# markkurossi/mpc

Measured on AMD Instinct MI355X. Metric: AND-gates/sec (garble+eval), AES-128 circuit batch, higher is better.
Workload: dtype u32 (AES T-table / 128-bit label XOR, integer); 1 GPU; aes_128.circ 36663 gates / 6400 AND, batch=1024 instances per GPU, 32-byte garbling key; instances_per_gpu=1024, levels=308, launches_per_garble=1, schedule=fused-flat, hash_phases=89, lds_live_labels=1053, graph=True, outputs_ok=True, device_memory=gc_dev_alloc / gc_dev_upload (C ABI); no torch in the process, gathers=0

## Files before the change

mpc_amd/csrc/plan.cpp:

```cpp
#include "plan.h"

#include <algorithm>
#include <chrono>
#include <cstdio>
#include <cstdlib>
#include <map>
#include <numeric>

namespace gc {

namespace {
struct PlanLaps {
    bool on = std::getenv("GC_TRACE") != nullptr;
    std::chrono::steady_clock::time_point t = std::chrono::steady_clock::now();
    void lap(const char *what) {
        if (!on) return;
        const auto n = std::chrono::steady_clock::now();
        std::fprintf(stderr, "[gc trace] plan: %-28s %8.3f ms\n", what, std::chrono::duration<double, std::milli>(n - t).count());
        t = n;
    }
};
}

static inline int op_class(uint8_t op) {
    switch (op) {
    case GC_AND: return 0;
    case GC_OR: return 1;
    case GC_INV: return 2;
    default: return 3;
    }
}


static void symdiff(const std::vector<uint32_t> &a, const std::vector<uint32_t> &b, std::vector<uint32_t> *o) {
    o->clear();
    size_t i = 0, j = 0;
    while (i < a.size() || j < b.size()) {
        if (j == b.size() || (i < a.size() && a[i] < b[j])) o->push_back(a[i++]);
        else if (i == a.size() || b[j] < a[i]) o->push_back(b[j++]);
        else i++, j++;
    }
}

namespace {
struct OpView {
    const uint8_t *ops;
    struct G {
        uint8_t op;
    };
    G operator[](uint32_t g) const { return G{ops[g]}; }
};
}

static void build_flat(const OpView gates, uint32_t ngates, uint32_t nwires, uint32_t ninputs, uint32_t noutputs,
                       const std::vector<uint32_t> &src0, const std::vector<uint32_t> &src1,
                       const std::vector<uint32_t> &cur, Plan *out, bool late = false) {
    Plan &p = *out;
    PlanLaps laps;
    const uint32_t NONE = 0xffffffffu;
    const uint32_t nprod = ninputs + ngates;
    std::vector<uint32_t> phase_of;
    if (late) {
        std::vector<uint32_t> early(nprod, 0);
        uint32_t last = 0;
        for (uint32_t g = 0; g < ngates; g++) {
            const uint32_t a = std::max(early[src0[g]], early[src1[g]]);
            early[ninputs + g] = op_class(gates[g].op) != 3 ? a + 1 : a;
            last = std::max(last, early[ninputs + g]);
        }
        std::vector<uint32_t> need_by(nprod, last);
        phase_of.assign(ngates, 0);
        for (uint32_t g = ngates; g-- > 0;) {
            const uint32_t pid = ninputs + g;
            uint32_t by = need_by[pid];
            if (op_class(gates[g].op) != 3) {
                phase_of[g] = std::max(by, early[pid]);
                by = phase_of[g] - 1;
            }
            need_by[src0[g]] = std::min(need_by[src0[g]], by);
            need_by[src1[g]] = std::min(need_by[src1[g]], by);
        }
    }
    std::vector<uint32_t> A(nprod, 0), Rr(nprod, 0);
    std::vector<uint8_t> is_free(nprod, 0), rpar(ngates, 0);
    std::vector<std::vector<uint32_t>> ex(ngates);
    std::map<std::vector<uint32_t>, uint32_t> sums;
    const bool two_level = std::getenv("GC_PLAN_NO_TWO_LEVEL") == nullptr;
    std::vector<uint32_t> t0, t1, tmp;
    std::vector<std::vector<uint32_t>> fx(ngates);
    std::vector<uint8_t> fdone(ngates, 0), fp(ngates, 0);
    std::vector<uint32_t> fstack, facc, fnxt, fsingles;
    auto full_of = [&](uint32_t top) {
        const uint32_t nreal = ninputs + ngates;
        fstack.assign(1, top);
        while (!fstack.empty()) {
            const uint32_t cur = fstack.back(), cg = cur - ninputs, ca = A[cur];
            if (fdone[cg]) {
                fstack.pop_back();
                continue;
            }
            auto own_c = [&](uint32_t t) { return t < nreal && is_free[t] && A[t] == ca; };
            bool ready = true;
            for (uint32_t t : ex[cg])
                if (own_c(t) && !fdone[t - ninputs]) fstack.push_back(t), ready = false;
            if (!ready) continue;
            fsingles.clear();
            for (uint32_t t : ex[cg])
                if (!own_c(t)) fsingles.push_back(t);
            facc.swap(fsingles);
            uint8_t par = rpar[cg];
            for (uint32_t t : ex[cg])
                if (own_c(t)) {
                    symdiff(facc, fx[t - ninputs], &fnxt);
                    facc.swap(fnxt);
                    par ^= fp[t - ninputs];
                }
            fx[cg] = facc;
            fp[cg] = par;
            fdone[cg] = 1;
            fstack.pop_back();
        }
    };
    for (uint32_t g = 0; g < ngates; g++) {
        const uint32_t pid = ninputs + g, s0 = src0[g], s1 = src1[g];
        const uint32_t a = std::max(A[s0], A[s1]);
        if (op_class(gates[g].op) != 3) {
            A[pid] = late ? phase_of[g] : a + 1;
            continue;
        }
        is_free[pid] = 1;
        A[pid] = a;
        auto rnd = [&](uint32_t s) { return (is_free[s] && A[s] == a) ? Rr[s] : 0u; };
        uint32_t r = std::max(std::max(rnd(s0), rnd(s1)), 1u);
        uint8_t par = gates[g].op == GC_XNOR;
        auto terms_of = [&](uint32_t s, std::vector<uint32_t> *t) {
            if (is_free[s] && A[s] == a && Rr[s] == r) {
                *t = ex[s - ninputs];
                par ^= rpar[s - ninputs];
            } else {
                t->assign(1, s);
            }
        };
        terms_of(s0, &t0);
        terms_of(s1, &t1);
        symdiff(t0, t1, &tmp);
        if (tmp.size() > kFlatMaxTerms && two_level) {
            const uint32_t nreal = ninputs + ngates;
            auto own = [&](uint32_t t) { return t < nreal && is_free[t] && A[t] == a; };
            std::vector<uint32_t> full, nxt;
            uint8_t fpar = par;
            for (uint32_t t : tmp)
                if (!own(t)) full.push_back(t);
            for (uint32_t t : tmp)
                if (own(t)) {
                    full_of(t);
                    symdiff(full, fx[t - ninputs], &nxt);
                    full.swap(nxt);
                    fpar ^= fp[t - ninputs];
                }
            std::vector<uint32_t> raw, rest;
            for (uint32_t t : full) ((t >= nreal && A[t] == a) ? rest : raw).push_back(t);
            const size_t nblocks = (raw.size() + kFlatMaxTerms - 1) / kFlatMaxTerms;
            if (rest.size() + nblocks <= kFlatMaxTerms) {
                for (size_t b0 = 0; b0 < raw.size(); b0 += kFlatMaxTerms) {
                    std::vector<uint32_t> blk(raw.begin() + (long)b0, raw.begin() + (long)std::min(raw.size(), b0 + kFlatMaxTerms));
                    if (blk.size() == 1) {
                        rest.push_back(blk[0]);
                        continue;
                    }
                    auto it = sums.find(blk);
                    if (it == sums.end() || A[it->second] > a) {
                        const uint32_t sp = (uint32_t)A.size();
                        A.push_back(a);
                        Rr.push_back(1);
                        is_free.push_back(1);
                        ex.push_back(blk);
                        rpar.push_back(0);
                        sums[blk] = sp;
                        it = sums.find(blk);
                    }
                    rest.push_back(it->second);
                }
                std::sort(rest.begin(), rest.end());
                size_t keep = 0;
                for (size_t i = 0; i < rest.size(); i++) {
                    if (i + 1 < rest.size() && rest[i] == rest[i + 1]) i++;
                    else rest[keep++] = rest[i];
                }
                rest.resize(keep);
                tmp.swap(rest);
                par = fpar;
                r = 2;
            }
        }
        if (tmp.size() > kFlatMaxTerms) {
            r += 1;
            par = gates[g].op == GC_XNOR;
            t0.assign(1, s0);
            t1.assign(1, s1);
            symdiff(t0, t1, &tmp);
        }
        Rr[pid] = r;
        rpar[g] = par;
        ex[g] = tmp;
    }
    laps.lap("flat: term lists");
    const uint32_t nprod2 = (uint32_t)A.size(), ngates2 = (uint32_t)ex.size();
    std::vector<uint8_t> need(nprod2, 0), is_output(nprod2, 0);
    std::vector<uint32_t> stack;
    for (uint32_t j = 0; j < noutputs; j++) {
        const uint32_t w = nwires - noutputs + j;
        if (cur[w] != NONE) {
            is_output[cur[w]] = 1;
            stack.push_back(cur[w]);
        }
    }
    for (uint32_t g = 0; g < ngates; g++)
        if (!is_free[ninputs + g]) {
            need[ninputs + g] = 1;
            stack.push_back(src0[g]);
            stack.push_back(src1[g]);
        }
    while (!stack.empty()) {
        const uint32_t s = stack.back();
        stack.pop_back();
        if (need[s] && (s < ninputs || !is_free[s])) continue;
        if (need[s]) continue;
        need[s] = 1;
        if (s >= ninputs && is_free[s])
            for (uint32_t t : ex[s - ninputs]) stack.push_back(t);
    }
    std::vector<uint32_t> gl;
    for (uint32_t g = 0; g < ngates2; g++)
        if (need[ninputs + g]) gl.push_back(g);
    auto key_of = [&](uint32_t g) { return ((uint64_t)A[ninputs + g] << 32) | ((uint64_t)Rr[ninputs + g] << 8); };
    auto sub_of = [&](uint32_t g) -> uint64_t {
        if (!is_free[ninputs + g]) return (uint64_t)op_class(gates[g].op);
        return 0xffu - std::min<uint64_t>(0xfeu, ex[g].size());
    };
    {
        std::vector<std::pair<uint64_t, uint32_t>> keyed(gl.size());
        for (size_t k = 0; k < gl.size(); k++) keyed[k] = {key_of(gl[k]) | sub_of(gl[k]), gl[k]};
        std::sort(keyed.begin(), keyed.end());
        for (size_t k = 0; k < gl.size(); k++) gl[k] = keyed[k].second;
    }
    std::vector<uint32_t> step_first;
    std::vector<uint32_t> step_of(ngates2, 0);
    for (uint32_t k = 0; k < gl.size(); k++) {
        if (k == 0 || key_of(gl[k]) != key_of(gl[k - 1])) step_first.push_back(k);
        step_of[gl[k]] = (uint32_t)step_first.size() - 1;
    }
    const uint32_t nsteps = (uint32_t)step_first.size();
    step_first.push_back((uint32_t)gl.size());
    p.n_flat_steps = nsteps;
    laps.lap("flat: needed + step order");
    std::vector<uint32_t> last_use(nprod2, 0);
    for (uint32_t g : gl) {
        const uint32_t st = step_of[g] + 1;
        if (is_free[ninputs + g]) {
            for (uint32_t t : ex[g]) last_use[t] = std::max(last_use[t], st);
        } else {
            last_use[src0[g]] = std::max(last_use[src0[g]], st);
            last_use[src1[g]] = std::max(last_use[src1[g]], st);
        }
    }
    std::vector<uint32_t> lds_of(nprod2, 0xffffu), free_list;
    std::vector<std::vector<uint32_t>> expire((size_t)nsteps + 2);
    uint32_t high = 0;
    auto take = [&]() {
        if (!free_list.empty()) {
            const uint32_t s = free_list.back();
            free_list.pop_back();
            return s;
        }
        return high++;
    };
    p.fl_in_lds.assign(ninputs, 0xffff);
    for (uint32_t w = 0; w < ninputs; w++) {
        if (last_use[w] == 0) continue;
        const uint32_t s = take();
        lds_of[w] = s;
        expire[last_use[w]].push_back(s);
    }
    for (uint32_t si = 0; si < nsteps; si++) {
        for (uint32_t s : expire[si]) free_list.push_back(s);
        for (uint32_t k = step_first[si]; k < step_first[si + 1]; k++) {
            const uint32_t pid = ninputs + gl[k];
            const uint32_t s = take();
            lds_of[pid] = s;
            expire[std::max(last_use[pid], si + 1)].push_back(s);
        }
    }
    if (std::getenv("GC_PLAN_DEBUG")) {
        std::vector<int32_t> delta((size_t)nsteps + 2, 0);
        uint32_t nin_live = 0;
        for (uint32_t w = 0; w < ninputs; w++)
            if (last_use[w]) nin_live++, delta[last_use[w]]--;
        for (uint32_t si = 0; si < nsteps; si++)
            for (uint32_t k = step_first[si]; k < step_first[si + 1]; k++) {
                const uint32_t pid = ninputs + gl[k];
                delta[si]++;
                delta[std::max(last_use[pid], si + 1)]--;
            }
        int32_t live = (int32_t)nin_live;
        std::fprintf(stderr, "[plan] %u steps, %u inputs live at start, high-water %u\n", nsteps, nin_live, high);
        for (uint32_t si = 0; si < nsteps; si++) {
            live += delta[si];
            std::fprintf(stderr, "[plan] step %u %s n=%u live=%d\n", si, is_free[ninputs + gl[step_first[si]]] ? "xor " : "hash",
                         step_first[si + 1] - step_first[si], live);
        }
    }
    const uint32_t zslot = high;
    if (high + 1 >= 0xffffu) {
        p.fl_in_lds.clear();
        return;
    }
    p.n_flat_slots = high + 1;
    for (uint32_t w = 0; w < ninputs; w++)
        if (lds_of[w] != 0xffffu) p.fl_in_lds[w] = (uint16_t)lds_of[w];

    laps.lap("flat: slots");
    std::vector<FDesc> uh;
    std::vector<XOut> uo;
    std::vector<uint32_t> uhg, uog;
    FUnit u{};
    u.xparts = 1;
    auto emit = [&]() {
        if (uh.empty() && uo.empty()) return;
        u.off16 = (uint32_t)(p.fl_prog.size() / 4);
        u.hfirst = (uint32_t)p.fl_hgslot.size();
        u.ofirst = (uint32_t)p.fl_ogslot.size();
        u.nout = (uint32_t)uo.size();
        for (const FDesc &d : uh) {
            p.fl_prog.push_back(d.lin);
            p.fl_prog.push_back(d.lout);
            p.fl_prog.push_back(d.tweak);
            p.fl_prog.push_back(d.row_op);
        }
        u.outs_off16 = (uint32_t)uh.size();
        {
            static const uint8_t grp_of[16] = {0, 1, 1, 0, 1, 0, 0, 1, 2, 3, 3, 2, 3, 2, 2, 3};
            for (size_t blk = 0; blk < uo.size(); blk += 16) {
                uint8_t used[4][8] = {};
                for (size_t o = blk; o < std::min(uo.size(), blk + 16); o++) {
                    XOut &x = uo[o];
                    uint8_t(&um)[8] = used[grp_of[o - blk]];
                    for (uint32_t k = 0; k < x.n; k++) {
                        uint32_t best = k;
                        for (uint32_t c = k; c < x.n; c++)
                            if (!(um[k] & (1u << (x.t[c] & 3)))) {
                                best = c;
                                break;
                            }
                        std::swap(x.t[k], x.t[best]);
                        um[k] |= (uint8_t)(1u << (x.t[k] & 3));
                    }
                    for (uint32_t k = x.n; k < (x.n > 4 ? 8u : 4u); k++) um[k] |= (uint8_t)(1u << (zslot & 3));
                }
            }
        }
        for (const XOut &x : uo) {
            for (int i = 0; i < 8; i += 2) p.fl_prog.push_back((uint32_t)x.t[i] | ((uint32_t)x.t[i + 1] << 16));
            p.fl_prog.push_back((uint32_t)x.out | ((uint32_t)x.flags << 16));
            p.fl_prog.push_back((uint32_t)x.n);
        }
        while (p.fl_prog.size() & 3) p.fl_prog.push_back(0);
        u.n16 = (uint32_t)(p.fl_prog.size() / 4) - u.off16;
        p.fl_hgslot.insert(p.fl_hgslot.end(), uhg.begin(), uhg.end());
        p.fl_ogslot.insert(p.fl_ogslot.end(), uog.begin(), uog.end());
        p.fl_units.push_back(u);
        p.fl_unit_stride = std::max(p.fl_unit_stride, (u.n16 + 3u) & ~3u);
        uh.clear(), uo.clear(), uhg.clear(), uog.clear();
        u = FUnit{};
        u.xparts = 1;
    };
    for (uint32_t si = 0; si < nsteps; si++) {
        const uint32_t k0 = step_first[si], k1 = step_first[si + 1];
        if (!is_free[ninputs + gl[k0]]) {
            emit();
            for (uint32_t k = k0; k < k1; k++) {
                if (uh.size() == kUHash) emit();
                const uint32_t g = gl[k], pid = ninputs + g;
                FDesc d;
                d.lin = lds_of[src0[g]] | (lds_of[src1[g]] << 16);
                d.lout = lds_of[pid] | (is_output[pid] ? kFStoreGlobal : 0u);
                d.tweak = p.tweak_of_gate[g];
                d.row_op = p.row_of_gate[g] | ((uint32_t)gates[g].op << kOpShift);
                uh.push_back(d);
                uhg.push_back(p.slot_of_gate[g]);
                if (gates[g].op == GC_AND) u.n_and++;
                else if (gates[g].op == GC_OR) u.n_or++;
                else u.n_inv++;
            }
        } else {
            if (!uo.empty()) emit();
            for (uint32_t k = k0; k < k1; k++) {
                const uint32_t g = gl[k], pid = ninputs + g;
                const uint32_t nt = (uint32_t)ex[g].size();
                const uint32_t P = nt <= 8 ? 1 : nt <= 16 ? 2 : 4;
                if (uo.size() + (P + 3) > kUOuts) emit();
                XOut dummy{};
                for (int i = 0; i < 8; i++) dummy.t[i] = (uint16_t)zslot;
                dummy.out = (uint16_t)zslot;
                dummy.flags = kXoPart;
                while (uo.size() % P) {
                    uo.push_back(dummy);
                    uog.push_back(0);
                }
                const uint32_t per = (nt + P - 1) / P;
                for (uint32_t part = 0; part < P; part++) {
                    const uint32_t lo = std::min(nt, per * part), hi = std::min(nt, per * (part + 1));
                    XOut x = dummy;
                    x.n = (uint16_t)(hi - lo);
                    for (uint32_t t = lo; t < hi; t++) x.t[t - lo] = (uint16_t)lds_of[ex[g][t]];
                    if (part == 0) {
                        x.out = (uint16_t)lds_of[pid];
                        x.flags = (uint16_t)((is_output[pid] ? kXoStore : 0) | (rpar[g] ? kXoRpar : 0) |
                                             (P == 2 ? kXoJoin2 : P == 4 ? kXoJoin4 : 0));
                    }
                    uo.push_back(x);
                    uog.push_back(part == 0 && g < ngates ? p.slot_of_gate[g] : 0);
                }
                u.xparts = std::max(u.xparts, P);
                p.fl_max_parts = std::max(p.fl_max_parts, P);
                p.n_flat_outs++;
                p.n_flat_terms += (uint32_t)ex[g].size();
            }
        }
    }
    emit();
    laps.lap("flat: units");
}

static void build_fused(const OpView gates, uint32_t ngates, uint32_t nwires, uint32_t ninputs, uint32_t noutputs,
                        const std::vector<uint32_t> &src0, const std::vector<uint32_t> &src1,
                        const std::vector<uint32_t> &cur, Plan *out) {
    Plan &p = *out;
    const uint32_t NONE = 0xffffffffu;
        const uint32_t nprod = ninputs + ngates;
        std::vector<uint32_t> ka(nprod, 0), kx(nprod, 0);
        std::vector<uint64_t> gkey(ngates);
        for (uint32_t g = 0; g < ngates; g++) {
            const uint32_t s0 = src0[g], s1 = src1[g];
            uint32_t a = ka[s0], x = kx[s0];
            if (ka[s1] > a || (ka[s1] == a && kx[s1] > x)) {
                a = ka[s1];
                x = kx[s1];
            }
            if (op_class(gates[g].op) != 3) {
                a += 1;
                x = 0;
            } else {
                x += 1;
            }
            ka[ninputs + g] = a;
            kx[ninputs + g] = x;
            gkey[g] = ((uint64_t)a << 40) | ((uint64_t)x << 8) | (uint64_t)op_class(gates[g].op);
        }
        std::vector<uint32_t> ford(ngates);
        {
            std::vector<std::pair<uint64_t, uint32_t>> keyed(ngates);
            for (uint32_t g = 0; g < ngates; g++) keyed[g] = {gkey[g], g};
            std::sort(keyed.begin(), keyed.end());
            for (uint32_t g = 0; g < ngates; g++) ford[g] = keyed[g].second;
        }
        std::vector<uint32_t> step_of_gate(ngates);
        for (uint32_t k = 0; k < ngates;) {
            const uint64_t key = gkey[ford[k]] >> 8;
            Step st{k, 0, 0, 0, 0, 0};
            while (k < ngates && (gkey[ford[k]] >> 8) == key) {
                const uint32_t g = ford[k];
                if (op_class(gates[g].op) != 3) st.nonfree++;
                if (gates[g].op == GC_AND) st.n_and++;
                else if (gates[g].op == GC_OR) st.n_or++;
                else if (gates[g].op == GC_INV) st.n_inv++;
                step_of_gate[g] = (uint32_t)p.fsteps.size();
                st.count++;
                k++;
            }
            if (st.nonfree) p.n_hash_phases++;
            p.fsteps.push_back(st);
        }
        const uint32_t NEVER = 0;
        std::vector<uint32_t> last_use(nprod, NEVER);
        for (uint32_t g = 0; g < ngates; g++) {
            const uint32_t st = step_of_gate[g] + 1;
            last_use[src0[g]] = std::max(last_use[src0[g]], st);
            last_use[src1[g]] = std::max(last_use[src1[g]], st);
        }
        std::vector<uint8_t> is_output(nprod, 0);
        for (uint32_t j = 0; j < noutputs; j++) {
            const uint32_t w = nwires - noutputs + j;
            if (cur[w] != NONE) is_output[cur[w]] = 1;
        }
        std::vector<uint32_t> lds_of(nprod, 0xffffu);
        std::vector<uint32_t> free_list;
        uint32_t high = 0;
        std::vector<std::vector<uint32_t>> expire(p.fsteps.size() + 2);
        auto take = [&]() {
            if (!free_list.empty()) {
                uint32_t s = free_list.back();
                free_list.pop_back();
                return s;
            }
            return high++;
        };
        p.in_lds.assign(ninputs, 0xffff);
        bool overflow = false;
        for (uint32_t w = 0; w < ninputs; w++) {
            if (last_use[w] == NEVER) continue;
            const uint32_t s = take();
            lds_of[w] = s;
            if (s >= 0xffff) overflow = true;
            else p.in_lds[w] = (uint16_t)s;
            expire[last_use[w]].push_back(s);
        }
        p.fdescs.resize(ngates);
        p.fgslot.resize(ngates);
        for (uint32_t si = 0, k = 0; si < p.fsteps.size(); si++) {
            for (uint32_t s : expire[si]) free_list.push_back(s);
            const Step &st = p.fsteps[si];
            for (uint32_t e = 0; e < st.count; e++, k++) {
                const uint32_t g = ford[k];
                const uint32_t pid = ninputs + g;
                const uint32_t s = take();
                if (s >= 0xffff) overflow = true;
                lds_of[pid] = s;
                const uint32_t lu = std::max(last_use[pid], si + 1);
                expire[lu].push_back(s);
                FDesc &d = p.fdescs[k];
                d.lin = (lds_of[src0[g]] & 0xffffu) | ((lds_of[src1[g]] & 0xffffu) << 16);
                d.lout = (s & 0xffffu) | (is_output[pid] ? kFStoreGlobal : 0u) | (e == 0 ? kFLevelStart : 0u);
                d.tweak = op_class(gates[g].op) == 3 ? si : p.tweak_of_gate[g];
                d.row_op = p.row_of_gate[g] | ((uint32_t)gates[g].op << kOpShift);
                p.fgslot[k] = p.slot_of_gate[g];
            }
        }
        p.n_lds_slots = overflow ? 0xffffffffu : high;
        Chunk ch{0, 0, 0, 0};
        for (uint32_t si = 0; si < p.fsteps.size(); si++) {
            const Step &st = p.fsteps[si];
            const bool cut = ch.nsteps && (st.nonfree || ch.ndesc + st.count > kChunkDescs || ch.nsteps == kChunkSteps);
            if (cut) {
                p.fchunks.push_back(ch);
                ch = Chunk{si, 0, st.first, 0};
            }
            ch.nsteps++;
            ch.ndesc += st.count;
        }
        if (ch.nsteps) p.fchunks.push_back(ch);

        p.info.n_hash_phases = p.n_hash_phases;
        p.info.n_fused_steps = (uint32_t)p.fsteps.size();
        p.info.n_lds_slots = p.n_lds_slots;
}

int simulate_flat(const Plan &p, const uint8_t *in_bits, uint8_t *out_bits) {
    if (p.n_flat_slots == 0xffffffffu) return GC_E_ARG;
    const uint32_t nin = p.info.ninputs;
    std::vector<uint8_t> lds(p.n_flat_slots, 0), glob(p.info.nslots, 0);
    std::vector<uint8_t> poison(p.n_flat_slots, 0);
    const uint32_t zslot = p.n_flat_slots - 1;
    poison[zslot] = 1;
    for (uint32_t w = 0; w < nin; w++) {
        glob[w] = in_bits[w] & 1;
        if (p.fl_in_lds[w] != 0xffff) lds[p.fl_in_lds[w]] = glob[w], poison[p.fl_in_lds[w]] = 1;
    }
    for (const FUnit &u : p.fl_units) {
        const uint32_t *img = p.fl_prog.data() + (size_t)u.off16 * 4;
        const uint32_t nh = u.n_and + u.n_or + u.n_inv;
        std::vector<std::pair<uint32_t, uint8_t>> writes;
        for (uint32_t g = 0; g < nh; g++) {
            const uint32_t lin = img[4 * g], lout = img[4 * g + 1], op = img[4 * g + 3] >> kOpShift;
            const uint32_t sa = lin & 0xffffu, sb = lin >> 16;
            if (!poison[sa] || (op != GC_INV && !poison[sb])) return GC_E_WIRE;
            if ((g < u.n_and) != (op == GC_AND) || (g >= u.n_and + u.n_or) != (op == GC_INV)) return GC_E_GATE;
            const uint8_t a = lds[sa], b = lds[sb];
            const uint8_t v = op == GC_AND ? (a & b) : op == GC_OR ? (a | b) : (uint8_t)(a ^ 1);
            writes.emplace_back(lout & 0xffffu, v);
            if (lout & kFStoreGlobal) glob[p.fl_hgslot[u.hfirst + g]] = v;
        }
        for (auto &w : writes) lds[w.first] = w.second, poison[w.first] = 1;
        writes.clear();
        const uint32_t *outs = img + (size_t)u.outs_off16 * 4;
        std::vector<uint8_t> partial(u.nout, 0);
        for (uint32_t o = 0; o < u.nout; o++) {
            const uint32_t *x = outs + 6 * o;
            const uint32_t n = x[5] & 0xffffu;
            uint8_t acc = 0;
            for (uint32_t k = 0; k < (n > 4 ? 8u : 4u); k++) {
                const uint32_t sl = (x[k / 2] >> (16 * (k & 1))) & 0xffffu;
                if (k < n ? !poison[sl] : sl != zslot) return GC_E_WIRE;
                acc ^= lds[sl];
            }
            partial[o] = acc;
        }
        for (uint32_t o = 0; o < u.nout; o++) {
            const uint32_t *x = outs + 6 * o;
            const uint32_t flags = x[4] >> 16, slot = x[4] & 0xffffu;
            if (flags & kXoPart) continue;
            uint8_t acc = partial[o];
            const uint32_t parts = (flags & kXoJoin4) ? 4u : (flags & kXoJoin2) ? 2u : 1u;
            if (parts > u.xparts || o % parts || o + parts > u.nout) return GC_E_ARG;
            for (uint32_t k = 1; k < parts; k++) {
                if (!((outs[6 * (o + k) + 4] >> 16) & kXoPart)) return GC_E_ARG;
                acc ^= partial[o + k];
            }
            if (flags & kXoRpar) acc ^= 1;
            writes.emplace_back(slot, acc);
            if (flags & kXoStore) glob[p.fl_ogslot[u.ofirst + o]] = acc;
        }
        for (auto &w : writes) lds[w.first] = w.second, poison[w.first] = 1;
    }
    for (uint32_t j = 0; j < p.info.noutputs; j++) out_bits[j] = glob[p.out_slots[j]];
    return GC_OK;
}

bool wide_for_one_instance(const Plan &p, bool eval) {
    const uint64_t passes = eval ? p.passes_eval : p.passes_garble;
    return p.levels.size() >= 2 && passes * 2 >= (uint64_t)p.levels.size() * 5;
}

void finish_flat(Plan *pp) {
    Plan &p = *pp;
    if (p.flat_built) return;
    PlanLaps laps;
    build_fused(OpView{p.lazy_ops.data()}, p.info.ngates, p.info.nwires, p.info.ninputs, p.info.noutputs, p.lazy_src0,
                p.lazy_src1, p.lazy_cur, &p);
    laps.lap("level-walking schedule");
    auto flat = [&](bool late) {
        p.fl_prog.clear(), p.fl_units.clear(), p.fl_hgslot.clear(), p.fl_ogslot.clear(), p.fl_in_lds.clear();
        p.n_flat_slots = 0xffffffffu;
        p.n_flat_outs = p.n_flat_terms = p.n_flat_steps = p.fl_unit_stride = 0;
        build_flat(OpView{p.lazy_ops.data()}, p.info.ngates, p.info.nwires, p.info.ninputs, p.info.noutputs, p.lazy_src0,
                   p.lazy_src1, p.lazy_cur, &p, late);
    };
    auto fits = [&]() {
        return p.n_flat_slots != 0xffffffffu &&
               ((size_t)kFlatStageOff16 + 2 * (size_t)p.fl_unit_stride + p.n_flat_slots + 1) * 16 <= kFlatLdsBytes;
    };
    const bool early_cannot_fit = p.n_lds_slots == 0xffffffffu || ((size_t)kFlatStageOff16 + p.n_lds_slots) * 16 > kFlatLdsBytes;
    const bool may_late = !std::getenv("GC_PLAN_NO_LATE");
    if (std::getenv("GC_PLAN_LATE")) {
        flat(true);
        p.flat_late = true;
    } else if (early_cannot_fit && may_late) {
        flat(true);
        p.flat_late = fits();
        if (!p.flat_late) flat(false);
    } else {
        flat(false);
        if (!fits() && may_late) {
            flat(true);
            p.flat_late = fits();
            if (!p.flat_late) flat(false);
        }
    }
    p.flat_built = true;
    p.info.n_flat_slots = p.n_flat_slots;
    p.info.n_flat_outs = p.n_flat_outs;
    p.info.n_flat_terms = p.n_flat_terms;
    p.info.n_flat_steps = p.n_flat_steps;
    p.info.n_flat_units = (uint32_t)p.fl_units.size();
    std::vector<uint8_t>().swap(p.lazy_ops);
    std::vector<uint32_t>().swap(p.lazy_src0);
    std::vector<uint32_t>().swap(p.lazy_src1);
    std::vector<uint32_t>().swap(p.lazy_cur);
}

int build_plan(const gc_gate *gates, uint32_t ngates, uint32_t nwires, uint32_t ninputs, uint32_t noutputs,
               Plan *out, bool defer_flat, const uint32_t *seg_first, uint32_t nseg) {
    if ((!gates && ngates) || !out) return GC_E_ARG;
    const bool tr__ = std::getenv("GC_TRACE") != nullptr;
    auto t__ = std::chrono::steady_clock::now();
    auto lap = [&](const char *what) {
        if (!tr__) return;
        const auto n = std::chrono::steady_clock::now();
        std::fprintf(stderr, "[gc trace] plan: %-28s %8.3f ms\n", what, std::chrono::duration<double, std::milli>(n - t__).count());
        t__ = n;
    };
    if (ninputs > nwires || noutputs > nwires) return GC_E_ARG;
    if ((uint64_t)ninputs + ngates >= 0xffffffffull) return GC_E_ARG;
    Plan &p = *out;
    p = Plan{};
    p.info.ngates = ngates;
    p.info.nwires = nwires;
    p.info.ninputs = ninputs;
    p.info.noutputs = noutputs;
    p.info.nslots = ninputs + ngates;

    const uint32_t NONE = 0xffffffffu;
    p.level_of_gate.resize(ngates);
    p.tweak_of_gate.resize(ngates);
    p.row_of_gate.resize((size_t)ngates + 1);
    p.slot_of_gate.resize(ngates);
    p.slot_of_wire.assign(nwires, NONE);
    for (uint32_t w = 0; w < ninputs; w++) p.slot_of_wire[w] = w;

    std::vector<uint32_t> wire_level(nwires, 0);
    std::vector<uint32_t> src0(ngates), src1(ngates);
    std::vector<uint32_t> cur(nwires, NONE);
    for (uint32_t w = 0; w < ninputs; w++) cur[w] = w;
    uint32_t id = 0, row = 0, max_level = 0, seg = 0;
    for (uint32_t g = 0; g < ngates; g++) {
        const gc_gate &G = gates[g];
        while (seg < nseg && seg_first[seg] <= g) {
            if (seg_first[seg] == g) id = 0;
            seg++;
        }
        if (G.op > GC_INV) return GC_E_GATE;
        const bool unary = (G.op == GC_INV);
        if (G.in0 >= nwires || G.out >= nwires || (!unary && G.in1 >= nwires)) return GC_E_WIRE;
        if (cur[G.in0] == NONE || (!unary && cur[G.in1] == NONE)) return GC_E_WIRE;
        uint32_t level = wire_level[G.in0];
        if (!unary) level = std::max(level, wire_level[G.in1]);
        p.level_of_gate[g] = level;
        src0[g] = cur[G.in0];
        src1[g] = unary ? cur[G.in0] : cur[G.in1];
        p.tweak_of_gate[g] = id;
        p.row_of_gate[g] = row;
        switch (G.op) {
        case GC_AND: id += 2; row += 2; p.info.n_and++; break;
        case GC_OR: id += 1; row += 3; p.info.n_or++; break;
        case GC_INV: id += 1; row += 1; p.info.n_inv++; break;
        case GC_XOR: p.info.n_xor++; break;
        default: p.info.n_xnor++; break;
        }
        if (row > kRowMask) return GC_E_ARG;
        wire_level[G.out] = level + 1;
        max_level = std::max(max_level, level + 1);
        cur[G.out] = ninputs + g;
    }
    p.row_of_gate[ngates] = row;
    p.info.slab_rows = row;
    p.info.nlevels = max_level;

    lap("pass 1");
    std::vector<uint32_t> order(ngates);
    {
        std::vector<uint32_t> start(((size_t)max_level + 1) * 4 + 1, 0);
        auto key_of = [&](uint32_t g) { return (size_t)p.level_of_gate[g] * 4 + (size_t)op_class(gates[g].op); };
        for (uint32_t g = 0; g < ngates; g++) start[key_of(g) + 1]++;
        for (size_t i = 1; i < start.size(); i++) start[i] += start[i - 1];
        for (uint32_t g = 0; g < ngates; g++) order[start[key_of(g)]++] = g;
    }
    lap("sort by level");
    for (uint32_t k = 0; k < ngates; k++) p.slot_of_gate[order[k]] = ninputs + k;
    auto slot_of_src = [&](uint32_t s) { return s < ninputs ? s : p.slot_of_gate[s - ninputs]; };

    p.descs.resize(ngates);
    p.gate_of_desc = order;
    uint32_t width = 0;
    for (uint32_t k = 0; k < ngates;) {
        uint32_t lvl = p.level_of_gate[order[k]];
        Step st{k, 0, 0, 0, 0, 0};
        while (k < ngates && p.level_of_gate[order[k]] == lvl) {
            uint32_t g = order[k];
            GateDesc &d = p.descs[k];
            d.in0 = slot_of_src(src0[g]);
            d.in1 = slot_of_src(src1[g]);
            d.tweak = p.tweak_of_gate[g];
            d.row_op = p.row_of_gate[g] | ((uint32_t)gates[g].op << kOpShift);
            if (op_class(gates[g].op) != 3) st.nonfree++;
            if (gates[g].op == GC_AND) st.n_and++;
            else if (gates[g].op == GC_OR) st.n_or++;
            else if (gates[g].op == GC_INV) st.n_inv++;
            st.count++;
            k++;
        }
        width = std::max(width, st.count);
        p.levels.push_back(st);
    }
    p.info.max_width = width;
    p.info.n_steps = (uint32_t)p.levels.size();

    for (uint32_t w = ninputs; w < nwires; w++)
        if (cur[w] != NONE) p.slot_of_wire[w] = slot_of_src(cur[w]);
    p.out_slots.resize(noutputs);
    for (uint32_t j = 0; j < noutputs; j++) {
        uint32_t s = p.slot_of_wire[nwires - noutputs + j];
        if (s == NONE) return GC_E_WIRE;
        p.out_slots[j] = s;
    }

    lap("descs + levels");
    lap("hash-phase schedule");
    for (const Step &st : p.levels) {
        const uint32_t fr = st.count - st.nonfree;
        p.passes_garble += (((st.n_and + st.n_or) << 2) + (st.n_inv << 1) + fr + 1023) / 1024;
        p.passes_eval += ((st.n_and << 1) + st.n_or + st.n_inv + fr + 1023) / 1024;
    }
    p.lazy_ops.resize(ngates);
    for (uint32_t g = 0; g < ngates; g++) p.lazy_ops[g] = gates[g].op;
    p.lazy_src0.swap(src0);
    p.lazy_src1.swap(src1);
    p.lazy_cur.swap(cur);
    p.info.n_flat_slots = 0xffffffffu;
    lap("lazy copies");
    if (!defer_flat) finish_flat(&p);
    lap("flat");
    return GC_OK;
}

}

extern "C" {

gc_plan *gc_plan_create(const gc_gate *gates, uint32_t ngates, uint32_t nwires, uint32_t ninputs,
                        uint32_t noutputs, int *status) try {
    gc_plan *pl = new (std::nothrow) gc_plan;
    int rc = pl ? gc::build_plan(gates, ngates, nwires, ninputs, noutputs, &pl->p) : GC_E_NOMEM;
    if (rc != GC_OK) {
        delete pl;
        pl = nullptr;
    }
    if (status) *status = rc;
    return pl;
} catch (...) {
    const int rc__ = gc::on_exception();
    if (status) *status = rc__;
    return nullptr;
}

void gc_plan_free(gc_plan *pl) { delete pl; }

int gc_plan_get_info(const gc_plan *pl, gc_plan_info *out) {
    if (!pl || !out) return GC_E_ARG;
    *out = pl->p.info;
    return GC_OK;
}

int gc_plan_simulate(const gc_plan *pl, const uint8_t *in_bits, uint8_t *out_bits) try {
    if (!pl || (!in_bits && pl->p.info.ninputs) || (!out_bits && pl->p.info.noutputs)) return GC_E_ARG;
    return gc::simulate_flat(pl->p, in_bits, out_bits);
} catch (...) {
    return gc::on_exception();
}

int gc_plan_fingerprint(const gc_plan *pl, uint64_t *fp) try {
    if (!pl || !fp) return GC_E_ARG;
    const gc::Plan &p = pl->p;
    uint64_t h = 14695981039346656037ull;
    auto mix = [&h](const void *data, size_t n) {
        const uint8_t *b = (const uint8_t *)data;
        for (size_t i = 0; i < n; i++) h = (h ^ b[i]) * 1099511628211ull;
        h = (h ^ (uint64_t)n) * 1099511628211ull;
    };
    auto vec = [&mix](const auto &v) { mix(v.data(), v.size() * sizeof(v[0])); };
    vec(p.descs), vec(p.levels), vec(p.out_slots);
    vec(p.fdescs), vec(p.fgslot), vec(p.fsteps), vec(p.fchunks), vec(p.in_lds);
    vec(p.fl_prog), vec(p.fl_units), vec(p.fl_hgslot), vec(p.fl_ogslot), vec(p.fl_in_lds);
    const uint32_t tail[8] = {p.n_flat_slots, p.n_flat_outs, p.n_flat_terms, p.n_flat_steps, p.flat_late ? 1u : 0u,
                              p.fl_unit_stride, p.fl_max_parts, p.n_lds_slots};
    mix(tail, sizeof tail);
    *fp = h;
    return GC_OK;
} catch (...) {
    return gc::on_exception();
}

int gc_plan_describe(const gc_plan *pl, uint32_t *level_of_gate, uint32_t *tweak_of_gate, uint32_t *row_of_gate,
                     uint32_t *slot_of_gate) try {
    if (!pl) return GC_E_ARG;
    const gc::Plan &p = pl->p;
    if (level_of_gate) std::copy(p.level_of_gate.begin(), p.level_of_gate.end(), level_of_gate);
    if (tweak_of_gate) std::copy(p.tweak_of_gate.begin(), p.tweak_of_gate.end(), tweak_of_gate);
    if (row_of_gate) std::copy(p.row_of_gate.begin(), p.row_of_gate.end(), row_of_gate);
    if (slot_of_gate) std::copy(p.slot_of_gate.begin(), p.slot_of_gate.end(), slot_of_gate);
    return GC_OK;
} catch (...) {
    return gc::on_exception();
}

}
```

mpc_amd/csrc/plan.h:

```cpp
#pragma once

#include <cstdint>
#include <vector>

#include "../../include/gcengine.h"

namespace gc {

int on_exception() noexcept;

struct GateDesc {
    uint32_t in0;
    uint32_t in1;
    uint32_t tweak;
    uint32_t row_op;
};
static_assert(sizeof(GateDesc) == 16, "GateDesc must be 16 bytes");

constexpr uint32_t kOpShift = 29;
constexpr uint32_t kRowMask = (1u << kOpShift) - 1;

struct Step {
    uint32_t first;
    uint32_t count;
    uint32_t nonfree;
    uint32_t n_and, n_or, n_inv;
};

struct FDesc {
    uint32_t lin;
    uint32_t lout;
    uint32_t tweak;
    uint32_t row_op;
};
static_assert(sizeof(FDesc) == 16, "FDesc must be 16 bytes");
constexpr uint32_t kFStoreGlobal = 1u << 16;
constexpr uint32_t kFLevelStart = 1u << 17;

constexpr uint32_t kChunkDescs = 768;
constexpr uint32_t kChunkSteps = 32;
struct Chunk {
    uint32_t first_step, nsteps;
    uint32_t first_desc, ndesc;
};

constexpr uint32_t kFlatMaxTerms = 32;
struct XOut {
    uint16_t t[8];
    uint16_t out;
    uint16_t flags;
    uint16_t n;
    uint16_t pad_;
};
static_assert(sizeof(XOut) == 24, "XOut must be 24 bytes");
constexpr uint16_t kXoStore = 1;
constexpr uint16_t kXoRpar = 2;
constexpr uint16_t kXoJoin2 = 4;
constexpr uint16_t kXoJoin4 = 8;
constexpr uint16_t kXoPart = 16;
constexpr uint32_t kUHash = 256, kUOuts = 448;
constexpr uint32_t kUnit16 = kUHash + kUOuts * 24 / 16;
struct FUnit {
    uint32_t off16, n16;
    uint32_t n_and, n_or, n_inv;
    uint32_t nout;
    uint32_t outs_off16;
    uint32_t xparts;
    uint32_t hfirst, ofirst;
    uint32_t pad_[2];
};
static_assert(sizeof(FUnit) == 48, "FUnit must be 48 bytes");

struct Plan {
    gc_plan_info info{};
    std::vector<uint32_t> level_of_gate, tweak_of_gate, row_of_gate , slot_of_gate;
    std::vector<GateDesc> descs;
    std::vector<uint32_t> gate_of_desc;
    std::vector<Step> levels;
    std::vector<uint32_t> slot_of_wire;
    std::vector<uint32_t> out_slots;

    std::vector<FDesc> fdescs;
    std::vector<uint32_t> fgslot;
    std::vector<Step> fsteps;
    std::vector<Chunk> fchunks;
    std::vector<uint32_t> fl_prog;
    std::vector<FUnit> fl_units;
    std::vector<uint32_t> fl_hgslot, fl_ogslot;
    std::vector<uint16_t> fl_in_lds;
    uint32_t n_flat_slots = 0xffffffffu;
    uint32_t n_flat_outs = 0, n_flat_terms = 0, n_flat_steps = 0;
    bool flat_late = false;
    uint32_t fl_unit_stride = 0;
    uint32_t fl_max_parts = 1;
    std::vector<uint16_t> in_lds;
    uint32_t n_lds_slots = 0;
    uint32_t n_hash_phases = 0;
    bool flat_built = false;
    std::vector<uint8_t> lazy_ops;
    std::vector<uint32_t> lazy_src0, lazy_src1, lazy_cur;
    uint32_t passes_garble = 0, passes_eval = 0;
};

int build_plan(const gc_gate *gates, uint32_t ngates, uint32_t nwires, uint32_t ninputs, uint32_t noutputs,
               Plan *out, bool defer_flat = false, const uint32_t *seg_first = nullptr, uint32_t nseg = 0);
void finish_flat(Plan *p);
bool wide_for_one_instance(const Plan &p, bool eval);

int simulate_flat(const Plan &p, const uint8_t *in_bits, uint8_t *out_bits);

constexpr uint32_t kFlatStageOff16 = 65536 / 16 + 16;
constexpr size_t kFlatLdsBytes = 160 * 1024;

}

struct gc_plan {
    gc::Plan p;
};
```

Measured before the change: 6.772 billion AND-gates/s.

## Reorder XOR terms per wave via bipartite matching to cut LDS bank conflicts

Replaces the greedy per-16-output term swap with a post-pass that, for each wave's block of flat outputs, permutes each output's XOR term slots so that lanes in the same group read distinct LDS banks per read position, using an augmenting-path matching with iterative refinement. The bank model depends on the instance-per-thread factor computed from LDS capacity, now exposed as flat_full_ti_log2. The simulator check is relaxed so zero-slot padding can sit anywhere among the real reads, as long as the non-zero count matches. This adds host-side planning time and depends on the bank model matching the hardware.

Measured after the change: 6.810 billion AND-gates/s (median of 6 runs). No clear change (+0.6%).

```diff
diff --git a/mpc_amd/csrc/plan.cpp b/mpc_amd/csrc/plan.cpp
--- a/mpc_amd/csrc/plan.cpp
+++ b/mpc_amd/csrc/plan.cpp
@@ -4,6 +4,7 @@
 #include <chrono>
 #include <cstdio>
 #include <cstdlib>
+#include <cstring>
 #include <map>
 #include <numeric>
 
@@ -50,6 +51,146 @@
     };
     G operator[](uint32_t g) const { return G{ops[g]}; }
 };
+}
+
+uint32_t flat_full_ti_log2(const Plan &p) {
+    uint32_t t = p.fl_max_parts >= 4 ? 2u : p.fl_max_parts == 2 ? 3u : 6u;
+    auto bytes = [&](uint32_t tt) {
+        return ((size_t)kFlatStageOff16 + 2 * (size_t)p.fl_unit_stride) * 16 + (((size_t)p.n_flat_slots + 1) << tt) * 16;
+    };
+    while (t > 0 && bytes(t) > kFlatLdsBytes) t--;
+    return t;
+}
+
+static void order_flat_terms(Plan *pp) {
+    Plan &p = *pp;
+    if (p.n_flat_slots == 0xffffffffu) return;
+    const uint32_t ti_log2 = flat_full_ti_log2(p), TI = 1u << ti_log2;
+    if (TI > 4) return;
+    const uint32_t cmask = 16 / TI - 1, per_wave = 64 / TI;
+    static const uint8_t grp_of_quad[16] = {0, 1, 1, 0, 1, 0, 0, 1, 2, 3, 3, 2, 3, 2, 2, 3};
+    constexpr uint32_t kKeys = 17;
+    uint8_t cn[4][8][16], worst[4][8];
+    static thread_local uint16_t ckey[4][8][16][kKeys];
+    for (const FUnit &u : p.fl_units) {
+        uint32_t *outs = p.fl_prog.data() + ((size_t)u.off16 + u.outs_off16) * 4;
+        for (uint32_t w0 = 0; w0 < u.nout; w0 += per_wave) {
+            const uint32_t w1 = std::min(u.nout, w0 + per_wave);
+            bool eight = false;
+            for (uint32_t o = w0; o < w1; o++) eight |= (outs[6 * o + 5] & 0xffffu) > 4;
+            const uint32_t nread = eight ? 8u : 4u;
+            auto group_of = [&](uint32_t o) { return (uint32_t)grp_of_quad[((o - w0) * TI) >> 2]; };
+            auto reset = [&](uint32_t g) {
+                std::memset(cn[g], 0, sizeof cn[g]);
+                std::memset(worst[g], 1, sizeof worst[g]);
+            };
+            auto claim = [&](uint32_t o) {
+                const uint32_t *x = outs + 6 * o, g = group_of(o);
+                for (uint32_t k = 0; k < nread; k++) {
+                    const uint16_t s = (uint16_t)((x[k / 2] >> (16 * (k & 1))) & 0xffffu);
+                    const uint32_t f = s & cmask;
+                    uint8_t &n = cn[g][k][f];
+                    bool have = false;
+                    for (uint32_t j = 0; j < n; j++) have |= ckey[g][k][f][j] == s;
+                    if (!have && n < kKeys) ckey[g][k][f][n++] = s;
+                    worst[g][k] = std::max(worst[g][k], n);
+                }
+            };
+            auto place = [&](uint32_t o) {
+                uint32_t *x = outs + 6 * o;
+                const uint32_t np = (x[5] & 0xffffu) > 4 ? 8u : 4u;
+                const uint32_t g = group_of(o);
+                uint16_t term[8];
+                for (uint32_t k = 0; k < 8; k++) term[k] = (uint16_t)((x[k / 2] >> (16 * (k & 1))) & 0xffffu);
+                auto cost = [&](uint16_t sl, uint32_t k) {
+                    const uint32_t f = sl & cmask, n = cn[g][k][f];
+                    if (!n) return 0u;
+                    bool have = false;
+                    for (uint32_t j = 0; j < n; j++) have |= ckey[g][k][f][j] == sl;
+                    return have ? 0u : n + 1u > worst[g][k] ? 2u + n : 1u;
+                };
+                bool free_as_is = true;
+                for (uint32_t k = 0; k < np && free_as_is; k++) free_as_is = cost(term[k], k) == 0;
+                if (free_as_is) return;
+                uint8_t cst[8][8], adj[2][8];
+                for (uint32_t i = 0; i < np; i++) {
+                    adj[0][i] = adj[1][i] = 0;
+                    if (i && term[i] == term[i - 1]) {
+                        for (uint32_t k = 0; k < np; k++) cst[i][k] = cst[i - 1][k];
+                        adj[0][i] = adj[0][i - 1], adj[1][i] = adj[1][i - 1];
+                        continue;
+                    }
+                    for (uint32_t k = 0; k < np; k++) {
+                        const uint32_t c = cost(term[i], k);
+                        cst[i][k] = (uint8_t)c;
+                        if (c == 0) adj[0][i] |= (uint8_t)(1u << k);
+                        if (c <= 1) adj[1][i] |= (uint8_t)(1u << k);
+                    }
+                }
+                int pos_of[8], term_at[8];
+                for (uint32_t i = 0; i < 8; i++) pos_of[i] = term_at[i] = -1;
+                uint32_t matched = 0;
+                for (uint32_t tier = 0; tier < 2 && matched < np; tier++) {
+                    const uint8_t *ad = adj[tier];
+                    for (uint32_t i = 0; i < np; i++) {
+                        if (pos_of[i] >= 0) continue;
+                        const uint8_t open = ad[i];
+                        if (!open) continue;
+                        struct Fr {
+                            uint32_t i;
+                            uint8_t left;
+                        } st[9];
+                        int via[8];
+                        uint8_t seen = 0;
+                        int sp = 0, found = -1;
+                        st[0] = Fr{i, open};
+                        while (sp >= 0 && found < 0) {
+                            Fr &fr = st[sp];
+                            const uint8_t cand = (uint8_t)(fr.left & ~seen);
+                            if (!cand) {
+                                sp--;
+                                continue;
+                            }
+                            const uint32_t k = (uint32_t)__builtin_ctz(cand);
+                            fr.left = (uint8_t)(fr.left & ~(1u << k));
+                            seen |= (uint8_t)(1u << k);
+                            via[k] = (int)fr.i;
+                            if (term_at[k] < 0) found = (int)k;
+                            else st[++sp] = Fr{(uint32_t)term_at[k], ad[term_at[k]]};
+                        }
+                        if (found >= 0) matched++;
+                        while (found >= 0) {
+                            const int t = via[found], prev = pos_of[t];
+                            pos_of[t] = found;
+                            term_at[found] = t;
+                            found = prev;
+                        }
+                    }
+                }
+                for (uint32_t i = 0; i < np && matched < np; i++) {
+                    if (pos_of[i] >= 0) continue;
+                    uint32_t best = 8, bc = 0;
+                    for (uint32_t k = 0; k < np; k++)
+                        if (term_at[k] < 0 && (best == 8 || cst[i][k] < bc)) best = k, bc = cst[i][k];
+                    pos_of[i] = (int)best;
+                    term_at[best] = (int)i;
+                    matched++;
+                }
+                uint16_t placed[8];
+                for (uint32_t k = 0; k < 8; k++) placed[k] = k < np ? term[term_at[k]] : term[k];
+                for (uint32_t k = 0; k < 8; k += 2) x[k / 2] = (uint32_t)placed[k] | ((uint32_t)placed[k + 1] << 16);
+            };
+            for (uint32_t g = 0; g < 4; g++) reset(g);
+            for (uint32_t o = w0; o < w1; o++) place(o), claim(o);
+            for (uint32_t o = w0, rounds = 2 * (w1 - w0); rounds--; o = o + 1 < w1 ? o + 1 : w0) {
+                const uint32_t g = group_of(o);
+                reset(g);
+                for (uint32_t q = w0; q < w1; q++)
+                    if (q != o && group_of(q) == g) claim(q);
+                place(o);
+            }
+        }
+    }
 }
 
 static void build_flat(const OpView gates, uint32_t ngates, uint32_t nwires, uint32_t ninputs, uint32_t noutputs,
@@ -338,27 +479,6 @@
             p.fl_prog.push_back(d.row_op);
         }
         u.outs_off16 = (uint32_t)uh.size();
-        {
-            static const uint8_t grp_of[16] = {0, 1, 1, 0, 1, 0, 0, 1, 2, 3, 3, 2, 3, 2, 2, 3};
-            for (size_t blk = 0; blk < uo.size(); blk += 16) {
-                uint8_t used[4][8] = {};
-                for (size_t o = blk; o < std::min(uo.size(), blk + 16); o++) {
-                    XOut &x = uo[o];
-                    uint8_t(&um)[8] = used[grp_of[o - blk]];
-                    for (uint32_t k = 0; k < x.n; k++) {
-                        uint32_t best = k;
-                        for (uint32_t c = k; c < x.n; c++)
-                            if (!(um[k] & (1u << (x.t[c] & 3)))) {
-                                best = c;
-                                break;
-                            }
-                        std::swap(x.t[k], x.t[best]);
-                        um[k] |= (uint8_t)(1u << (x.t[k] & 3));
-                    }
-                    for (uint32_t k = x.n; k < (x.n > 4 ? 8u : 4u); k++) um[k] |= (uint8_t)(1u << (zslot & 3));
-                }
-            }
-        }
         for (const XOut &x : uo) {
             for (int i = 0; i < 8; i += 2) p.fl_prog.push_back((uint32_t)x.t[i] | ((uint32_t)x.t[i + 1] << 16));
             p.fl_prog.push_back((uint32_t)x.out | ((uint32_t)x.flags << 16));
@@ -430,6 +550,8 @@
     }
     emit();
     laps.lap("flat: units");
+    order_flat_terms(&p);
+    laps.lap("flat: term order");
 }
 
 static void build_fused(const OpView gates, uint32_t ngates, uint32_t nwires, uint32_t ninputs, uint32_t noutputs,
@@ -588,11 +710,18 @@
             const uint32_t *x = outs + 6 * o;
             const uint32_t n = x[5] & 0xffffu;
             uint8_t acc = 0;
-            for (uint32_t k = 0; k < (n > 4 ? 8u : 4u); k++) {
+            uint32_t nreal = 0;
+            for (uint32_t k = 0; k < 8; k++) {
                 const uint32_t sl = (x[k / 2] >> (16 * (k & 1))) & 0xffffu;
-                if (k < n ? !poison[sl] : sl != zslot) return GC_E_WIRE;
+                if (k >= (n > 4 ? 8u : 4u)) {
+                    if (sl != zslot) return GC_E_WIRE;
+                    continue;
+                }
+                if (!poison[sl]) return GC_E_WIRE;
+                nreal += sl != zslot;
                 acc ^= lds[sl];
             }
+            if (nreal != n) return GC_E_WIRE;
             partial[o] = acc;
         }
         for (uint32_t o = 0; o < u.nout; o++) {
diff --git a/mpc_amd/csrc/plan.h b/mpc_amd/csrc/plan.h
--- a/mpc_amd/csrc/plan.h
+++ b/mpc_amd/csrc/plan.h
@@ -107,6 +107,8 @@
 void finish_flat(Plan *p);
 bool wide_for_one_instance(const Plan &p, bool eval);
 
+uint32_t flat_full_ti_log2(const Plan &p);
+
 int simulate_flat(const Plan &p, const uint8_t *in_bits, uint8_t *out_bits);
 
 constexpr uint32_t kFlatStageOff16 = 65536 / 16 + 16;
```
